# juhyeonkim95/Mitsuba3DopplerToF

Measured on AMD Instinct MI355X. Metric: Mpaths/s (whole node), Doppler Cornell 512x512 64spp, higher is better.
Workload: dtype f32

## Files before the change

mitsuba3dopplertof_amd/csrc/dtof_device.h:

```cpp
#pragma once
#include "dtof_kernels.h"
#include "dtof_scene.h"
#include "dtof_math.h"

#define DTOF_D __device__ __forceinline__
namespace dtof { constexpr int kBlock = 256; }
#include "dtof_traverse.h"
#include "dtof_sampling.h"
#include "dtof_shading.h"

#include <stdexcept>
#include <cstdlib>

namespace dtof {

constexpr uint32_t kSeg = 512;
static_assert(kSeg / 64 == kChunkBlocks, "chunks per segment");
constexpr int kShadeBlock = 64;
static_assert(kShadeBlock == 64, "k_shade's compaction (wave_append) and its per-wave statistics take the block for one wave");
template <bool MESH> DTOF_D void store_hit(const Queues &q, uint32_t l, const Hit &h, bool found) {
    if (MESH) q.hit[l] = make_uint4(f2u(h.t), f2u(h.u), f2u(h.v), h.prim);
    else q.hit_t[l] = h.t;
    q.hit_id[l] = found ? (h.obj | (h.shape << q.id_shift)) : 0xffffffffu;
}
template <bool MESH> DTOF_D uint4 load_hit(const Queues &q, uint32_t l) {
    if (MESH) return q.hit[l];
    return make_uint4(f2u(q.hit_t[l]), 0u, 0u, 0u);
}
DTOF_D uint32_t seg_count(const uint32_t *counts, uint32_t seg, uint32_t n_lanes) {
    return counts ? counts[seg] : min(kSeg, n_lanes - seg * kSeg);
}

DTOF_D float tent(float x, float inv_r) { return fmax_(0.f, 1.f - fabsf(x * inv_r)); }
template <int F = -1>
DTOF_D float filter_weight(const RenderParams &rp, float x) {
    const int filter = F >= 0 ? F : (int) rp.filter;
    if (filter == FILTER_GAUSSIAN) return fmax_(estrin10(sqr(x), rp.gauss_coeff), 0.f);
    if (filter == FILTER_MITCHELL) {
        x = fabsf(x);
        const float x2 = x * x, x3 = x2 * x, B = rp.filter_b, C = rp.filter_c;
        const float a3 = (12.f - 9.f * B - 6.f * C), a2 = (-18.f + 12.f * B + 6.f * C), a0 = (6.f - 2.f * B),
                    b3 = (-B - 6.f * C), b2 = (6.f * B + 30.f * C), b1 = (-12.f * B - 48.f * C), b0 = (8.f * B + 24.f * C);
        const float r = (1.f / 6.f) * (x < 1.f ? fmaf(a3, x3, fmaf(a2, x2, a0)) : fmaf(b3, x3, fmaf(b2, x2, fmaf(b1, x, b0))));
        return x < 2.f ? r : 0.f;
    }
    if (filter == FILTER_CATMULLROM) {
        x = fabsf(x);
        const float x2 = x * x, x3 = x2 * x, B = 0.f, C = .5f;
        const float r = (1.f / 6.f) * (x < 1.f ? (12.f - 9.f * B - 6.f * C) * x3 + (-18.f + 12.f * B + 6.f * C) * x2 + (6.f - 2.f * B)
                                               : (-B - 6.f * C) * x3 + (6.f * B + 30.f * C) * x2 + (-12.f * B - 48.f * C) * x + (8.f * B + 24.f * C));
        return x < 2.f ? r : 0.f;
    }
    if (filter == FILTER_LANCZOS) {
        x = fabsf(x);
        const float x1 = kPi * x, x2 = x1 / rp.filter_radius;
        float s1, s2, c; sincos_(x1, s1, c); sincos_(x2, s2, c);
        const float result = (s1 * s2) / (x1 * x2);
        return x < 5.9604644775390625e-8f ? 1.f : (x > rp.filter_radius ? 0.f : result);
    }
    return tent(x, rp.inv_radius);
}
template <int CTRL, int ROW_MASK = 0xf>
DTOF_D float dpp_add(float v) {
    return v + __int_as_float(__builtin_amdgcn_update_dpp(0, __float_as_int(v), CTRL, ROW_MASK, 0xf, false));
}

template <int F = -1>
DTOF_D void splat_lane(const RenderParams &rp, float *film, float spx, float spy, int pixel_x, int pixel_y, float r, float g, float b) {
    int W = rp.crop_w, H = rp.crop_h;
    if (F >= 0 ? F == FILTER_BOX : rp.filter == FILTER_BOX) {
        int x = pixel_x, y = pixel_y;
        if ((unsigned) x < (unsigned) W && (unsigned) y < (unsigned) H) {
            float *p = film + 4 * ((size_t) y * W + x);
            atomicAdd(p, r); atomicAdd(p + 1, g); atomicAdd(p + 2, b); atomicAdd(p + 3, 1.f);
        }
        return;
    }
    int n = (int) ceilf(rp.filter_radius - .5f), cnt = 2 * n + 1;
    int pix = (int) floorf(spx) - n, piy = (int) floorf(spy) - n;
    float relx = (float) pix + .5f - spx, rely = (float) piy + .5f - spy;
    int lx = pix - rp.crop_x, ly = piy - rp.crop_y;
    for (int ys = 0; ys < cnt; ++ys) {
        float wy = filter_weight<F>(rp, rely + (float) ys);
        for (int xs = 0; xs < cnt; ++xs) {
            float w = filter_weight<F>(rp, relx + (float) xs) * wy;
            int x = lx + xs, y = ly + ys;
            if ((unsigned) x < (unsigned) W && (unsigned) y < (unsigned) H) {
                float *p = film + 4 * ((size_t) y * W + x);
                atomicAdd(p, r * w); atomicAdd(p + 1, g * w); atomicAdd(p + 2, b * w); atomicAdd(p + 3, w);
            }
        }
// ... 35 lines not shown
```

mitsuba3dopplertof_amd/csrc/dtof_kernels.h:

```cpp
#pragma once
#include <stdint.h>
#include <hip/hip_runtime.h>
#include "dtof_math.h"

namespace dtof {

constexpr uint32_t kChunkBlocks = 8;
constexpr uint32_t kMaxInline = 4;
constexpr int kMaxOffsets = 4;

struct RenderParams {
    float s2c[16];
    float cam_to_world[12];
    float near_clip, far_clip, shutter_open, shutter_open_time;
    int32_t orthographic;
    float aperture_radius, focus_distance;
    int32_t crop_x, crop_y, crop_w, crop_h;
    float scale_x, scale_y, offset_x, offset_y;
    int32_t filter; float filter_radius, inv_radius;
    float gauss_coeff[10];
    float filter_b, filter_c;
    uint32_t base_seed, seed, seed_value;
    uint32_t spp, spp_log2;
    uint32_t tcn, pcn;
// ... 51 lines not shown
    uint32_t *q[2];
    uint32_t *counts;
    uint4 *cand;
    uint32_t *defer_idx;
    uint32_t *defer_cnt;
    uint32_t *seg_counter;
    uint32_t capacity;
    uint32_t xcd_remap;
    uint32_t id_shift;
};

struct LaneDebug {
    float sample_pos[2]; float time; float ray_o[3]; float ray_d[3]; float rgb[3]; float valid;
};

struct ShadeArgs {
    const uint8_t *scene; uint32_t scene_bytes, stage_words; RenderParams rp; Queues q;
    const uint32_t *qin, *count_in; uint32_t *qout, *alive_out, *shadow_out; uint32_t depth, trace_next; LaneDebug *dbg;
    float *film; uint64_t film_stride;
    uint32_t n_seg, res_small_off, res_small_words, res_memo;
    uint32_t res_park_off;
};
static_assert(sizeof(ShadeArgs) == 888, "ShadeArgs is k_shade's kernarg block: its layout, order and types do not change");
constexpr uint32_t kParkWords = 11;
#ifndef DTOF_PARK
#define DTOF_PARK 1
#endif
constexpr uint32_t kParkState = 10, kParkRng = 6;
constexpr uint32_t kResidentNodes = 1024;
constexpr uint32_t kMemoStride = 64, kMemoWords = 12;

struct ShadeLds {
    uint32_t stage, memo;
    uint32_t stack, park;
    constexpr uint32_t bytes() const { return stage + memo + stack + park; }
    constexpr uint32_t without_stack() const { return stage + memo + park; }
    constexpr uint32_t park_off() const { return stack / 4u; }
    static constexpr ShadeLds columns(uint32_t stage_words, uint32_t waves, uint32_t memo_columns, uint32_t stack_depth, bool entries16, uint32_t park_words) {
        return { stage_words * 16u, memo_columns * waves * kMemoWords * kMemoStride * 4u, (stack_depth < 2 ? 2u : stack_depth) * waves * 64u * (entries16 ? 2u : 4u), park_words * waves * 64u * 4u };
    }
    static constexpr ShadeLds classic(uint32_t stage_words, bool fused, bool one_instance, uint32_t stack_depth) {
        return fused ? columns(stage_words, 1u, one_instance ? 2u : 1u, one_instance ? 1u : stack_depth, false, 0u) : ShadeLds { stage_words * 16u, 0u, 0u, 0u };
    }
    static constexpr ShadeLds resident(uint32_t small_words, uint32_t waves, bool memo, bool several_films, uint32_t stack_depth) {
        return columns(4u * kResidentNodes + small_words, waves, memo ? 1u : 0u, stack_depth, several_films, (several_films ? kParkWords : 0u) + (DTOF_PARK && waves == 16 ? (several_films ? kParkRng : kParkState) : 0u));
    }
};
static_assert(ShadeLds::resident(171, 16, false, false, 12).bytes() == 158384 && ShadeLds::resident(171, 16, true, false, 12).bytes() == 207536, "resident stage, one film");
static_assert(ShadeLds::resident(171, 8, false, true, 12).bytes() == 103088 && ShadeLds::resident(171, 8, false, true, 12).park_off() == 3072, "resident stage, four films");
static_assert(ShadeLds::classic(214, true, true, 5).bytes() == 10080 && ShadeLds::classic(214, true, true, 5).without_stack() == 9568, "classic one-wall launch");

enum : uint32_t {
    kFactSinglePass     = 1u << 0,
    kFactDopplerCorr    = 1u << 1,
    kFactNoLaneOutput   = 1u << 2,
    kFactIdentityQueue  = 1u << 3,
    kFactNoRoulette     = 1u << 4,
    kFactCorrelated     = 1u << 5,
    kFactWholePath      = 1u << 6,
    kFactOneBlock       = 1u << 7,
    kFactOneEmitter     = 1u << 8,
    kFactWavePixel      = 1u << 9,
    kFactFlat           = 1u << 10,
    kFactOneWall        = 1u << 11,
    kFactFusedSplat     = 1u << 12,
};
#ifndef DTOF_HEADLINE_FACTS
#define DTOF_HEADLINE_FACTS 0xfff
#endif
constexpr uint32_t kHeadlineFacts = DTOF_HEADLINE_FACTS;
#ifndef DTOF_HEADLINE_FUSED
#define DTOF_HEADLINE_FUSED 1
#endif
constexpr uint32_t kHeadlineFusedFacts = DTOF_HEADLINE_FUSED ? (kHeadlineFacts | kFactFusedSplat) : 0u;
#ifndef DTOF_WALL_FRAMES
#define DTOF_WALL_FRAMES 1
#endif
#ifndef DTOF_RESIDENT_FACTS
#define DTOF_RESIDENT_FACTS 0x37f
#endif
constexpr uint32_t kResidentFacts = DTOF_RESIDENT_FACTS;

struct ShadeLaunch { bool staged; int mode; uint32_t waves, grid, lds, lds_flat; hipStream_t stream; ShadeArgs args; uint32_t facts; };
bool launch_shade_plain(bool area, bool k4, const ShadeLaunch &L);
void launch_shade_mesh(bool area, bool k4, const ShadeLaunch &L);
void launch_shade_spec1(bool k4, const ShadeLaunch &L);
void launch_shade_spec2(bool k4, const ShadeLaunch &L);
bool launch_shade_resident0(bool area, bool k4, const ShadeLaunch &L);
void launch_shade_resident1(bool k4, const ShadeLaunch &L);
void launch_shade_resident2(bool k4, const ShadeLaunch &L);

struct ResidentStage { uint32_t small_off = 0, small_words = 0, waves = 0, n_cu = 0; };
inline ShadeLds resident_lds(const RenderParams &rp, const ResidentStage &st, uint32_t stack_depth, uint32_t waves) { return ShadeLds::resident(st.small_words, waves, rp.memo_obj != 0xffffffffu, rp.n_offsets != 1, stack_depth); }
uint32_t device_lds_limit();
uint32_t device_cu_count();

struct LaunchSwitches {
// ... 60 lines not shown
```

mitsuba3dopplertof_amd/csrc/dtof_sampling.h:

```cpp
#pragma once
#include "dtof_kernels.h"
#include "dtof_scene.h"
#include "dtof_math.h"

#ifndef DTOF_D
#define DTOF_D __device__ __forceinline__
#endif

namespace dtof {

struct Rng { uint64_t state, inc; };
DTOF_D float next_f32(Rng &r) { return pcg_next_f32(r.state, r.inc); }
DTOF_D Rng seed_stream(uint32_t seed_value, uint32_t index) {
    uint32_t v0, v1; tea32(seed_value, index, v0, v1);
    Rng r; pcg_seed(v0, v1, r.state, r.inc); return r;
}
DTOF_D uint64_t stream_inc(uint32_t seed_value, uint32_t index) {
    uint32_t v0, v1; tea32(seed_value, index, v0, v1);
    return ((uint64_t) v1 << 1) | 1u;
}
DTOF_D float next_correlate(Rng &main, Rng &path, bool correlate) {
    uint64_t old = correlate ? path.state : main.state;
    path.state = path.state * kPcgMult + path.inc;
    main.state = main.state * kPcgMult + main.inc;
    return pcg_output_f32(old);
}
DTOF_D float next_time(const RenderParams &rp, Rng &main, Rng &tm, uint32_t si, uint32_t perm_seed, uint32_t &dim) {
    int strategy = rp.time_sampling; uint32_t tcn = rp.tcn;
    if (strategy == TIME_UNIFORM) return next_f32(main);
    float r = strategy == TIME_STRATIFIED ? next_f32(main) : next_f32(tm);
    const uint32_t quo = fdiv(si, rp.d_tcn), rem = si - quo * tcn;
    if (rp.stratify) {
        if (strategy == TIME_STRATIFIED) {
            const uint32_t ps = perm_seed + dim + ((rem != 0) ? 0u : 1u);
            dim += 2;
            const uint32_t p = permute_kensler(quo, rp.n_stratum, ps, rp.d_stratum);
            r = ((float) p + r) * rp.inv_n_stratum;
        } else {
            r = ((float) quo + r) * rp.inv_n_stratum;
        }
    }
    if (strategy == TIME_STRATIFIED) return ((float) rem + r) * rp.inv_tcn;
    if (strategy == TIME_ANTITHETIC) {
        if (tcn == 2) { float r2 = r + rp.antithetic_shift; return rem != 1 ? r : r2; }
        return r + (float) rem / (float) tcn;
    }
    if (strategy == TIME_ANTITHETIC_MIRROR) {
        float r2 = 1.0f - r + rp.antithetic_shift;
        return rem != 1 ? r : r2;
    }
    if (strategy == TIME_PERIODIC) return r + (float) rem / (float) tcn;
    return r;
}

constexpr float kInvTwoPiF = 0.15915494309189533577f;
DTOF_D float waveform(float _t, int type) {
    float t = fmod_pos(_t, 2.f * kPi, kInvTwoPiF);
    if (type == WAVE_RECT) return fabsf(t - kPi) > 0.5f * kPi ? 1.f : -1.f;
    if (type == WAVE_TRI) return t < kPi ? 1.f - 2.f * t * (1.0f / kPi) : -3.f + 2.f * t * (1.0f / kPi);
    return cos_(t);
}
DTOF_D float waveform_low_pass(float _t, int type) {
    float t = fmod_pos(_t, 2.f * kPi, kInvTwoPiF);
    if (type == WAVE_SIN) return cos_(t);
    float a = t * (1.0f / kPi), b = 2.f - a, c = a < b ? a : b;
    if (type == WAVE_RECT) return 2.f - 4.f * c;
    if (type == WAVE_TRI) return (4.f * c * c * c - 6.f * c * c + 1.f) * 2.0f * (1.0f / 3.0f);
    float r = 2.f - 4.f * c;
    return fmin_(fmax_(2.0f * r, -2.0f), 2.0f);
}
DTOF_D float modulation_weight(const RenderParams &rp, float w_d, float phase, float ray_time, float path_length) {
    float phi = rp.phi_coef * path_length;
    if (rp.low_pass) {
        float t = w_d * ray_time + phase + phi;
        return rp.amp * waveform_low_pass(t, rp.wave_type);
    }
    float t1 = rp.w_g * ray_time - phi;
    float t2 = (rp.w_g + w_d) * ray_time + phase;
    float g_t = rp.g_1 * waveform(t1, rp.wave_type) + rp.g_0;
    float s_t = waveform(t2, rp.wave_type);
    return s_t * g_t;
}

struct PrimaryLane { float4 ray_a, ray_b; Rng main, path; float2 pos; };
DTOF_D uint32_t global_lane(const RenderParams &rp, uint32_t virtual_lane) {
    if (rp.stripe_rows == 0) return virtual_lane;
    const uint32_t v = fdiv(virtual_lane, rp.d_lanes_per_row), in_row = virtual_lane - v * rp.lanes_per_row;
    const uint32_t s = fdiv(v, rp.d_stripe_rows), y = rp.stripe_first + s * rp.stripe_period + (v - s * rp.stripe_rows);
    return y * rp.lanes_per_row + in_row;
}
struct PixelInfo { uint32_t perm_seed; float posx, posy; };
template <bool UNIFORM>
DTOF_D PixelInfo pixel_info(const RenderParams &rp, uint32_t pix) {
    if (UNIFORM) pix = __builtin_amdgcn_readfirstlane(pix);
    PixelInfo pi; uint32_t tmp;
    tea32(rp.base_seed, rp.spp * pix + rp.seed, pi.perm_seed, tmp);
    const uint32_t W = (uint32_t) rp.crop_w, py = fdiv(pix, rp.d_w), px = pix - W * py;
    pi.posx = (float) (px + (uint32_t) rp.crop_x); pi.posy = (float) (py + (uint32_t) rp.crop_y);
    return pi;
}
template <bool PERSPECTIVE_ONLY = false>
DTOF_D void camera_ray(const RenderParams &rp, float ax, float ay, float apx, float apy, V3 &o, V3 &dw, float &maxt) {
    const float *m = rp.s2c;
    float r0 = fmaf(m[2], 0.f, fmaf(m[1], ay, fmaf(m[0], ax, m[3])));
    float r1 = fmaf(m[6], 0.f, fmaf(m[5], ay, fmaf(m[4], ax, m[7])));
    float r2 = fmaf(m[10], 0.f, fmaf(m[9], ay, fmaf(m[8], ax, m[11])));
    float r3 = fmaf(m[14], 0.f, fmaf(m[13], ay, fmaf(m[12], ax, m[15])));
    float iw = rcp(r3);
    V3 near_p = mk(r0 * iw, r1 * iw, r2 * iw);
    if (!PERSPECTIVE_ONLY && rp.orthographic) {
        o = xf_point(rp.cam_to_world, near_p);
        dw = normalize(xf_vector(rp.cam_to_world, mk(0.f, 0.f, 1.f)));
        maxt = rp.far_clip - rp.near_clip;
        return;
    }
    const bool lens = !PERSPECTIVE_ONLY && rp.aperture_radius != 0.f;
    V3 d;
    if (lens) {
        float tx, ty; concentric_disk(apx, apy, tx, ty);
        const V3 aperture_p = mk(rp.aperture_radius * tx, rp.aperture_radius * ty, 0.f);
        const float f_dist = rp.focus_distance / near_p.z;
        d = normalize(near_p * f_dist - aperture_p);
        o = xf_point(rp.cam_to_world, aperture_p);
    } else {
        d = normalize(near_p);
        o = mk(rp.cam_to_world[3], rp.cam_to_world[7], rp.cam_to_world[11]);
    }
    dw = xf_vector(rp.cam_to_world, d);
    float inv_z = rcp(d.z), near_t = rp.near_clip * inv_z, far_t = rp.far_clip * inv_z;
    o = o + dw * near_t;
    maxt = far_t - near_t;
}

template <bool PERSPECTIVE_ONLY = false, uint32_t FACTS = 0>
DTOF_D PrimaryLane generate_lane(const RenderParams &rp, uint32_t lane, bool wave_pixel = false, uint32_t vlane = 0) {
    constexpr bool F_SINGLE_PASS = (FACTS & kFactSinglePass) != 0, F_DOPPLER_CORR = (FACTS & kFactDopplerCorr) != 0, F_CORRELATED = (FACTS & kFactCorrelated) != 0;
    const bool needs_tm = (F_DOPPLER_CORR || (rp.integrator == 0 && rp.sampler_kind == SAMPLER_CORRELATED)) && rp.time_sampling >= TIME_ANTITHETIC;
    Rng main, tm, path; tm.state = 0; tm.inc = 1;
    uint2 *const carried = !F_SINGLE_PASS && rp.n_passes > 1 ? rp.pass_rng + (size_t) (vlane - rp.pass_first) * 3 : nullptr;
    const uint32_t pass = F_SINGLE_PASS ? 0u : rp.pass;
    if (pass == 0 && wave_pixel && needs_tm && rp.tcn == 2 && rp.pcn == 2) {
        main = seed_stream(rp.seed_value, lane);
        const bool odd = lane & 1u;
        uint32_t a0, a1; tea32(rp.seed_value + (odd ? 2u : 1u), lane >> 1, a0, a1);
        const uint32_t b0 = (uint32_t) __builtin_amdgcn_update_dpp(0, (int) a0, 0xb1, 0xf, 0xf, false), b1 = (uint32_t) __builtin_amdgcn_update_dpp(0, (int) a1, 0xb1, 0xf, 0xf, false);
        pcg_seed(odd ? b0 : a0, odd ? b1 : a1, tm.state, tm.inc);
        pcg_seed(odd ? a0 : b0, odd ? a1 : b1, path.state, path.inc);
    } else if (pass == 0) {
        main = seed_stream(rp.seed_value, lane);
        if (needs_tm) tm = seed_stream(rp.seed_value + 1, fdiv(lane, rp.d_tcn));
        path = seed_stream(rp.seed_value + 2, fdiv(lane, rp.d_pcn));
    } else {
        const uint2 a = carried[0], b = carried[1], c = carried[2];
        main.state = (uint64_t) a.x | ((uint64_t) a.y << 32); main.inc = stream_inc(rp.seed_value, lane);
        if (needs_tm) { tm.state = (uint64_t) b.x | ((uint64_t) b.y << 32); tm.inc = stream_inc(rp.seed_value + 1, fdiv(lane, rp.d_tcn)); }
        path.state = (uint64_t) c.x | ((uint64_t) c.y << 32); path.inc = stream_inc(rp.seed_value + 2, fdiv(lane, rp.d_pcn));
    }
    const uint32_t pix = fdiv(lane, rp.d_spp);
// ... 41 lines not shown
```

mitsuba3dopplertof_amd/csrc/dtof_shade.h:

```cpp
#pragma once
#include "dtof_device.h"
#include <atomic>
#include <initializer_list>
#include <type_traits>

namespace dtof {


DTOF_D uint32_t wave_append(bool pred, uint32_t &running) {
    const uint64_t mask = __ballot(pred);
    const uint32_t slot = running + (uint32_t) __popcll(mask & ((1ull << __lane_id()) - 1ull));
    running += (uint32_t) __popcll(mask);
    return slot;
}

struct BsdfOut { V3 val, weight, wo; float pdf, bs_pdf, bs_eta; bool bs_delta, bs_null; };
template <int SPEC>
DTOF_D void bsdf_eval_pdf_sample(const SceneView &sv, const DShape *sh, Surface &si, V3 wo, bool active_em, float sample_1, float s2x, float s2y, BsdfOut &out, bool want_sample = true) {
    const bool masked = SPEC && (sh->flags & SF_MASK);
    bool null_pick = false; float opacity = 1.f;
    if (masked) { opacity = mask_opacity_at(sv, sh, si.u, si.v); null_pick = !(sample_1 < opacity); sample_1 = sample_1 / opacity; }
    const bool blend = SPEC == 2 && (sh->flags & SF_BLEND);
    float blend_w = 0.f; bool pick_1 = false;
    if (blend) {
        blend_w = sh->tex_blend ? texture_eval_1(sv, sh->tex_blend << 4, si.u, si.v) : sh->blend_weight;
        blend_w = fmin_(fmax_(blend_w, 0.f), 1.f);
        pick_1 = sample_1 <= blend_w;
    }
    const DShape *side_sh = (SPEC == 2 && (sh->flags & SF_TWOSIDED2) && si.wi.z < 0.f) ? &sv.shapes[sh->blend_other] : sh;
    const V3 wi_plain = si.wi, wo_plain = wo;
    V3 bsdf_val = mk(0, 0, 0), bsdf_weight = mk(0, 0, 0), bs_wo = mk(0, 0, 0);
    float bsdf_pdf = 0.f, bs_pdf = 0.f, bs_eta = 0.f; bool bs_delta = false, bs_null = false;
    V3 val_0 = mk(0, 0, 0), keep_weight = mk(0, 0, 0), keep_wo = mk(0, 0, 0); float pdf_0 = 0.f, keep_pdf = 0.f, keep_eta = 0.f; bool keep_delta = false, keep_null = false;
    for (int pass = 0; pass < (SPEC == 2 && blend ? 2 : 1); ++pass) {
        const DShape *bsh = pass ? &sv.shapes[sh->blend_other] : side_sh;
        const float s1 = !blend ? sample_1 : (pass ? sample_1 / blend_w : (sample_1 - blend_w) / (1.f - blend_w));
        si.wi = wi_plain; wo = wo_plain;
// ... 228 lines not shown
    w[9] = bo.bs_delta ? 1.f : 0.f; w[10] = bo.weight.x; w[11] = bo.weight.y; w[12] = bo.weight.z; w[13] = bo.bs_null ? 1.f : 0.f;
}
template <int SPEC>
void launch_bsdf_eval_spec(const uint8_t *scene, uint32_t shape_index, const float *in, float *out, uint32_t n, hipStream_t s) {
    if (n) hipLaunchKernelGGL(k_bsdf_eval<SPEC>, dim3(nblk(n)), dim3(kBlock), 0, s, scene, shape_index, in, out, n);
}

template <bool LDS, int MODE, bool AREA, int KMAX, bool MESH, int SPEC, int RESW = 0, bool RH16 = false, uint32_t FACTS = 0>
#ifndef DTOF_MESH_WAVES
#define DTOF_MESH_WAVES 3
#endif
#ifndef DTOF_K4_RES_LDS
#define DTOF_K4_RES_LDS 1
#endif
__global__ __launch_bounds__(RESW ? RESW * 64 : kShadeBlock, RESW ? RESW / 4 : (MODE == 2 && !MESH && !SPEC && KMAX == 1) ? 4 : (MODE != 0 && MESH) ? ((SPEC && KMAX > 1) ? 2 : DTOF_MESH_WAVES) : 1) void k_shade(ShadeArgs args_by_value) {
    constexpr bool FUSED = MODE != 0, FIRST = MODE == 2;
    static_assert(FACTS == 0 || MODE == 2, "plan facts describe a first-bounce launch");
    constexpr bool F_SINGLE_PASS = (FACTS & kFactSinglePass) != 0, F_DOPPLER_CORR = (FACTS & kFactDopplerCorr) != 0, F_NO_LANE_OUT = (FACTS & kFactNoLaneOutput) != 0;
    constexpr bool F_IDENTITY = (FACTS & kFactIdentityQueue) != 0, F_NO_RR = (FACTS & kFactNoRoulette) != 0, F_CORRELATED = (FACTS & kFactCorrelated) != 0;
    constexpr bool F_WHOLE_PATH = (FACTS & kFactWholePath) != 0, F_ONE_BLOCK = (FACTS & kFactOneBlock) != 0, F_ONE_EMITTER = (FACTS & kFactOneEmitter) != 0;
    constexpr bool F_WAVE_PIXEL = (FACTS & kFactWavePixel) != 0;
    constexpr bool F_FLAT = (FACTS & kFactFlat) != 0, F_ONE_WALL = (FACTS & kFactOneWall) != 0, F_FUSED_SPLAT = (FACTS & kFactFusedSplat) != 0;
    constexpr bool F_FRAMES = F_ONE_WALL && DTOF_WALL_FRAMES;
    static_assert(!F_FLAT || (!MESH && SPEC == 0 && RESW == 0), "trace_flat serves the staged rectangle-only diffuse kernels");
    static_assert(!F_ONE_WALL || F_FLAT, "the one wall is an object of the flat table");
    static_assert(!F_FUSED_SPLAT || KMAX == 1, "the fused splat is the one-film kernels'");
    static_assert(!F_WAVE_PIXEL || F_IDENTITY, "whole waves of one pixel are provable for an identity queue only");
    static_assert(!F_ONE_BLOCK || RESW == 0, "blocks per segment belong to the classic launch");
    constexpr bool RES_LDS = RESW != 0 && KMAX > 1 && DTOF_K4_RES_LDS;
    constexpr bool S16 = RESW != 0 && KMAX > 1;
    static_assert(!RES_LDS || 3 * KMAX == (int) kParkWords + 1, "the film-state columns hold all but the last float of the K results");
    constexpr bool PARK_ST = DTOF_PARK && RESW == 16 && KMAX == 1;
    constexpr bool PARK = DTOF_PARK && RESW == 16 && (KMAX == 1 || RES_LDS);
    constexpr uint32_t kRngAt = RES_LDS ? kParkWords : 0u;
    constexpr int KREG = RES_LDS ? 1 : KMAX;
    constexpr uint32_t kStackStride = RESW ? RESW * 64 : kShadeBlock;
    static_assert(RESW == 0 || (MODE == 2 && !LDS && MESH), "the resident stage exists for the unstaged fused first-bounce kernel with mesh code");
    static_assert(!RH16 || RESW != 0, "half-float LDS planes belong to the resident stage");
    extern __shared__ uint4 lds[];
    __shared__ uint32_t s_inline_all[(RESW ? RESW : 1) * 2 * kMaxInline];
    typedef const char __attribute__((address_space(4))) *KernargBytes;
    const KernargBytes kernarg = (KernargBytes) __builtin_amdgcn_kernarg_segment_ptr();
    const ShadeArgs &A0 = *(const ShadeArgs *) kernarg;
    const uint32_t lane_id = RESW ? threadIdx.x & 63u : threadIdx.x, wave_id = RESW ? threadIdx.x >> 6 : 0u;
    uint32_t *const s_inline = s_inline_all + wave_id * 2 * kMaxInline;
    const uint32_t stage_words = RESW ? 4u * kResNodes + A0.res_small_words : A0.stage_words;
// ... 29 lines not shown
        sv_res = make_view(A0.scene);
        sv_res.nodes = (const DNode *) lds; sv_res.nodes16 = (const DNode16 *) lds;
        sv_res.groups = (const DGroup *) (small + gh->off_groups); sv_res.shapes = (const DShape *) (small + gh->off_shapes);
        sv_res.tris = (const DTri *) (small + gh->off_tris); sv_res.shading = (const DTriShade *) (small + gh->off_shading);
        sv_res.isect = (const DTriIsect *) (small + gh->off_isect);
        sv_res.emitters = (const DEmitter *) (small + gh->off_emitters);
    }
    for (;;) {
    uint32_t seg, sub_index = 0;
    if (RESW) {
        uint32_t taken = 0;
        if (lane_id == 0) taken = atomicAdd(A0.q.seg_counter, 1u);
        uint32_t unit = (uint32_t) __builtin_amdgcn_readfirstlane((int) taken);
        if (unit >= A0.n_seg * sub) break;
        unit = A0.n_seg * sub - 1u - unit;
        seg = sub > 1 ? unit / sub : unit; sub_index = sub > 1 ? unit - seg * sub : 0u;
    } else {
        seg = sub > 1 ? blockIdx.x / sub : blockIdx.x; sub_index = sub > 1 ? blockIdx.x - seg * sub : 0u;
    }
    const uint32_t count = seg_count(F_IDENTITY ? nullptr : A0.count_in, seg, A0.rp.n_lanes);
    uint32_t n_alive = 0, n_shadow = 0;
    if (FIRST && lane_id < 2 * kMaxInline) s_inline[lane_id] = 0;
    if (count != 0) {
    const uint8_t *base = LDS ? stage_scene(A0.scene, A0.scene_bytes, lds) : A0.scene;
    SceneView sv = RESW ? sv_res : make_view(base);
    if (FUSED) { sv.memo_obj = A0.rp.memo_obj; sv.memo = (float *) (lds + stage_words) + (RESW ? wave_id * kMemoWords * kMemoStride + lane_id : threadIdx.x); sv.memo_m = memo_m_lds; }
    const bool have_memo = F_ONE_WALL || (FUSED && sv.memo_obj != 0xffffffffu);
    for (uint32_t cbase = sub > 1 ? sub_index * unit_lanes : 0u; cbase < (sub > 1 ? (sub_index + 1) * unit_lanes < count ? (sub_index + 1) * unit_lanes : count : count); cbase += kShadeBlock) {
    uint32_t rebase = 0;
    asm volatile("" : "+s"(rebase));
    const ShadeArgs &A = *(const ShadeArgs *) (kernarg + rebase);
    const RenderParams &rp = A.rp; const Queues &q = A.q;
    const uint32_t *const qin = F_IDENTITY ? nullptr : A.qin; uint32_t *const qout = A.qout; const uint32_t depth0 = A.depth, trace_next_last = F_WHOLE_PATH ? 0u : A.trace_next;
    LaneDebug *const dbg = F_NO_LANE_OUT ? nullptr : A.dbg;
    const uint32_t flat = FUSED && !MESH ? rp.flat_objects : 0u;
    uint32_t j = cbase + lane_id;
    bool in_range = F_WAVE_PIXEL || j < count;
    bool alive = false, want_shadow = false;
    uint32_t l = 0;
    float4 sha = make_float4(0.f, 0.f, 0.f, 0.f), shb = sha, nra = sha, nrb = sha; float3 cand[KREG];
#pragma unroll
    for (int k = 0; k < KREG; ++k) cand[k] = make_float3(0.f, 0.f, 0.f);
    float3 rbase[KREG];
#pragma unroll
    for (int k = 0; k < KREG; ++k) rbase[k] = make_float3(0.f, 0.f, 0.f);
    V3 pend_thr = mk(0, 0, 0), pend_v = mk(0, 0, 0); float pend_len = 0.f;
    float *const park = RES_LDS || PARK ? (float *) (lds + stage_words) + memo_words + A0.res_park_off + threadIdx.x : nullptr;
    float res_last = 0.f;
    auto res_get = [&](int k) -> float4 {
        if (RES_LDS) return make_float4(park[(3 * k) * kStackStride], park[(3 * k + 1) * kStackStride], 3 * k + 2 < (int) kParkWords ? park[(3 * k + 2) * kStackStride] : res_last, 0.f);
        if (!FIRST) return q.res[(size_t) k * q.capacity + l];
        const float3 r = rbase[k]; return make_float4(r.x, r.y, r.z, 0.f);
    };
    auto res_put = [&](int k, float4 v) {
        if (RES_LDS) {
// ... 25 lines not shown
    };
    const bool valid_start = SPEC && rp.has_env && !rp.hide_emitters;
    bool valid_reg = valid_start;
    float memo_m[12], memo_inv[12];
    typename std::conditional<F_FRAMES, WallFrames, NoFrames>::type wf;
    if constexpr (F_FRAMES) {
        wf.n = mk(0.f, 0.f, 1.f); wf.s = mk(1.f, 0.f, 0.f);
        wf.table = (const DFlatFrame *) ((const uint4 *) ((const DFlatObject *) (sv.base + rp.flat_off) + rp.flat_objects) + 1 + rp.flat_objects);
    }
    bool lane_on = in_range;
#ifdef DTOF_TRAVERSAL_STATS
    constexpr uint64_t kPoisonState = 0xdeadbeefcafef00dull;
    if (!in_range) { main.state = path.state = kPoisonState; const float pz = u2f(0x7fc0dead); ra = rb = st = make_float4(pz, pz, pz, pz); }
#define DTOF_POISON_CHECK() do { if (main.state == kPoisonState || path.state == kPoisonState || f2u(st.x) == 0x7fc0deadu || f2u(ra.x) == 0x7fc0deadu) DTOF_STAT(14); } while (0)
#else
#define DTOF_POISON_CHECK() ((void) 0)
#endif
    const bool wave_pixel = F_WAVE_PIXEL || (FIRST && rp.spp_log2 != 0xffffffffu && rp.spp_log2 >= 6 && (rp.lane_base & 63u) == 0 && count - cbase >= (uint32_t) kShadeBlock);
    const bool fuse_splat = F_FUSED_SPLAT || (FIRST && A.film != nullptr);
    float2 pos_reg = make_float2(0.f, 0.f);
    if (in_range) {
        l = qin ? qin[seg * kSeg + j] : seg * kSeg + j;
        if (FIRST) {
            const PrimaryLane pl = generate_lane<SPEC == 0, FACTS>(rp, global_lane(rp, rp.lane_base + l), wave_pixel, rp.lane_base + l);
            ra = pl.ray_a; rb = pl.ray_b; main = pl.main; path = pl.path; st = make_float4(1.f, 1.f, 1.f, 0.f);
            if (PARK) park_store();
            pos_reg = pl.pos;
            if (!fuse_splat) {
                q.pos[l] = pl.pos;
                q.rng_b[l] = make_uint2((uint32_t) (main.inc >> 1), (uint32_t) (path.inc >> 1));
            }
            if (dbg) {
                LaneDebug &o = dbg[l];
                o.time = ra.w; o.ray_o[0] = ra.x; o.ray_o[1] = ra.y; o.ray_o[2] = ra.z; o.ray_d[0] = rb.x; o.ray_d[1] = rb.y; o.ray_d[2] = rb.z;
            }
            if (have_memo) instance_memo_fill(sv, ra.w, memo_m, memo_inv);
            if constexpr (F_FRAMES) {
                const DShape &ws = sv.shapes[sv.groups[sv.objects[sv.memo_obj].index].first_shape];
                wf.n = normalize(xf_normal(memo_inv, mk(ws.n[0], ws.n[1], ws.n[2])));
                const V3 du = xf_vector(memo_m, mk(ws.dp_du[0], ws.dp_du[1], ws.dp_du[2]));
                wf.s = normalize(vfma(wf.n, -dot(wf.n, du), du));
                if (du.x == 0.f && du.y == 0.f && du.z == 0.f) { V3 tt; coordinate_system(wf.n, wf.s, tt); }
            }
            Hit h;
            bool found = (F_FLAT || flat) ? trace_flat<false, true, FACTS & kFactOneWall>(sv, (ConstBytes) A.scene + rp.flat_off, rp.flat_off, flat, stack, mk(ra.x, ra.y, ra.z), mk(rb.x, rb.y, rb.z), ra.w, rb.w, h)
                              : trace_scene<false, MESH, FUSED, RESW != 0, kStackStride, S16, 0u, false, RH16>(sv, stack, mk(ra.x, ra.y, ra.z), mk(rb.x, rb.y, rb.z), ra.w, rb.w, h);
            hh = make_uint4(f2u(h.t), f2u(h.u), f2u(h.v), h.prim);
// ... 360 lines not shown
        if (alive && trace_next) {
            Hit h;
            bool found = (F_FLAT || flat) ? trace_flat<false, true, FACTS & kFactOneWall>(sv, (ConstBytes) A.scene + rp.flat_off, rp.flat_off, flat, stack, mk(nra.x, nra.y, nra.z), mk(nrb.x, nrb.y, nrb.z), nra.w, nrb.w, h)
                              : trace_scene<false, MESH, true, RESW != 0, kStackStride, S16, 0u, false, RH16>(sv, stack, mk(nra.x, nra.y, nra.z), mk(nrb.x, nrb.y, nrb.z), nra.w, nrb.w, h);
            if (!FIRST || last) store_hit<MESH>(q, l, h, found);
            if (FIRST) { hh = make_uint4(f2u(h.t), f2u(h.u), f2u(h.v), h.prim); hid = found ? (h.obj | (h.shape << q.id_shift)) : 0xffffffffu; }
        }
        const uint32_t n_sh = (uint32_t) __popcll(__ballot(want_shadow)) * ((threadIdx.x & 63) == 0 ? 1u : 0u);
        if (last) n_shadow += n_sh; else if (lane_id == 0) s_inline[2 * it + 1] += n_sh;
    } else {
        uint32_t sslot = seg * kSeg + wave_append(want_shadow, n_shadow);
        if (want_shadow) {
            q.sh_a[sslot] = sha; q.sh_b[sslot] = shb;
#pragma unroll
            for (int k = 0; k < KMAX; ++k) if (KMAX == 1 || k < rp.n_offsets)
                q.sh_c[(size_t) k * q.capacity + sslot] = make_float4(cand[k].x, cand[k].y, cand[k].z, u2f(l));
        }
    }
    if (last) break;
    lane_on = alive;
    if (alive) { ra = nra; rb = nrb; DTOF_POISON_CHECK(); }
    }
    if constexpr (!RES_LDS) if (FIRST && fuse_splat) {
        const uint32_t W = (uint32_t) rp.crop_w;
        const uint32_t pix = fdiv(global_lane(rp, rp.lane_base + l), rp.d_spp);
        const int py = (int) fdiv(pix, rp.d_w), px = (int) (pix - W * (uint32_t) py);
        const float sx = pos_reg.x, sy = pos_reg.y;
        const bool regular = in_range && (int) floorf(sx) - rp.crop_x == px && (int) floorf(sy) - rp.crop_y == py;
        if (wave_pixel) {
            const int upx = __builtin_amdgcn_readfirstlane(px), upy = __builtin_amdgcn_readfirstlane(py);
            const float relx = (float) (upx + rp.crop_x - 1) + .5f - sx, rely = (float) (upy + rp.crop_y - 1) + .5f - sy;
            float wx[3], wy[3];
#pragma unroll
            for (int a = 0; a < 3; ++a) { wx[a] = regular ? tent(relx + (float) a, rp.inv_radius) : 0.f; wy[a] = tent(rely + (float) a, rp.inv_radius); }
            const uint32_t sum_id = __brev(lane_id) >> 26, tap = sum_id >> 2, ch = sum_id & 3u;
            const int fx = upx - 1 + (int) (tap % 3u), fy = upy - 1 + (int) (tap / 3u);
            const bool store = sum_id < 36u && (unsigned) fx < W && (unsigned) fy < (unsigned) rp.crop_h;
#pragma unroll
            for (int k = 0; k < KMAX; ++k) if (KMAX == 1 || k < rp.n_offsets) {
                float *fk = A.film + (size_t) k * A.film_stride;
                if (in_range && !regular) splat_lane<F_FUSED_SPLAT ? FILTER_TENT : -1>(rp, fk, sx, sy, px, py, rbase[k].x, rbase[k].y, rbase[k].z);
                float v[36];
#pragma unroll
                for (int ys = 0; ys < 3; ++ys)
#pragma unroll
                    for (int xs = 0; xs < 3; ++xs) {
                        const float w = wx[xs] * wy[ys]; const int c = 4 * (3 * ys + xs);
                        v[c] = rbase[k].x * w; v[c + 1] = rbase[k].y * w; v[c + 2] = rbase[k].z * w; v[c + 3] = w;
                    }
                const float total = wave_totals_36(v, lane_id);
                if (store && total != 0.f) atomicAdd(fk + 4 * ((size_t) fy * W + (size_t) fx) + ch, total);
            }
        } else if (in_range) {
#pragma unroll
            for (int k = 0; k < KMAX; ++k) if (KMAX == 1 || k < rp.n_offsets)
                splat_lane<F_FUSED_SPLAT ? FILTER_TENT : -1>(rp, A.film + (size_t) k * A.film_stride, sx, sy, px, py, rbase[k].x, rbase[k].y, rbase[k].z);
        }
    }
    }
    }
    if (lane_id == 0) {
        if (sub > 1) { atomicAdd(&A0.alive_out[seg], n_alive); atomicAdd(&A0.shadow_out[seg], n_shadow); }
        else { A0.alive_out[seg] = n_alive; A0.shadow_out[seg] = n_shadow; }
        if (FIRST) {
            const uint32_t n_inl = A0.rp.inline_iters, n_seg = RESW ? A0.n_seg : gridDim.x / sub;
            for (uint32_t i = 0; i + 1 < n_inl; ++i) {
                uint32_t *slot = A0.alive_out - (size_t) 2 * (n_inl - 1 - i) * n_seg;
                if (sub > 1) { atomicAdd(&slot[seg], s_inline[2 * i]); atomicAdd(&slot[n_seg + seg], s_inline[2 * i + 1]); }
                else { slot[seg] = s_inline[2 * i]; slot[n_seg + seg] = s_inline[2 * i + 1]; }
            }
        }
    }
    if (!RESW) break;
    }
#undef DTOF_POISON_CHECK
}

template <bool A, int K, bool M, int S>
static void launch_shade_variant(const ShadeLaunch &L) {
// ... 29 lines not shown
```

Baseline: 16070.

## Stage headline launch constants into LDS block with compile-time defaults

Adds a compact HeadlineConsts struct that the headline k_shade kernels copy from the kernarg RenderParams into shared memory at block start, with many rarely varying fields fixed as static constexpr values. Ray generation, bounce shading and the fused splat read from this block, so the compiler can fold the constant fields and drop the dead branches. It also moves per-pixel values into scalar registers through readfirstlane. The cost is one extra LDS staging pass and 432 B of static LDS per block, plus the risk of wrong output if any constexpr default does not match the real parameters.

After: 15640. -2.7%, worse.

```diff
diff --git a/mitsuba3dopplertof_amd/csrc/dtof_device.h b/mitsuba3dopplertof_amd/csrc/dtof_device.h
--- a/mitsuba3dopplertof_amd/csrc/dtof_device.h
+++ b/mitsuba3dopplertof_amd/csrc/dtof_device.h
@@ -32,8 +32,8 @@
 }
 
 DTOF_D float tent(float x, float inv_r) { return fmax_(0.f, 1.f - fabsf(x * inv_r)); }
-template <int F = -1>
-DTOF_D float filter_weight(const RenderParams &rp, float x) {
+template <int F = -1, class RP>
+DTOF_D float filter_weight(const RP &rp, float x) {
     const int filter = F >= 0 ? F : (int) rp.filter;
     if (filter == FILTER_GAUSSIAN) return fmax_(estrin10(sqr(x), rp.gauss_coeff), 0.f);
     if (filter == FILTER_MITCHELL) {
@@ -65,8 +65,8 @@
     return v + __int_as_float(__builtin_amdgcn_update_dpp(0, __float_as_int(v), CTRL, ROW_MASK, 0xf, false));
 }
 
-template <int F = -1>
-DTOF_D void splat_lane(const RenderParams &rp, float *film, float spx, float spy, int pixel_x, int pixel_y, float r, float g, float b) {
+template <int F = -1, class RP>
+DTOF_D void splat_lane(const RP &rp, float *film, float spx, float spy, int pixel_x, int pixel_y, float r, float g, float b) {
     int W = rp.crop_w, H = rp.crop_h;
     if (F >= 0 ? F == FILTER_BOX : rp.filter == FILTER_BOX) {
         int x = pixel_x, y = pixel_y;
diff --git a/mitsuba3dopplertof_amd/csrc/dtof_kernels.h b/mitsuba3dopplertof_amd/csrc/dtof_kernels.h
--- a/mitsuba3dopplertof_amd/csrc/dtof_kernels.h
+++ b/mitsuba3dopplertof_amd/csrc/dtof_kernels.h
@@ -97,6 +97,31 @@
     uint32_t res_park_off;
 };
 static_assert(sizeof(ShadeArgs) == 888, "ShadeArgs is k_shade's kernarg block: its layout, order and types do not change");
+
+struct alignas(16) HeadlineConsts {
+    float s2c[16], cam_to_world[12], near_clip, far_clip, shutter_open, shutter_open_time;
+    int32_t crop_x, crop_y, crop_w, crop_h; float scale_x, scale_y, offset_x, offset_y; int32_t filter; float filter_radius, inv_radius; uint32_t pad_film;
+    uint32_t base_seed, seed, seed_value, spp, spp_log2, tcn, pcn; int32_t time_sampling; float antithetic_shift; int32_t stratify; uint32_t n_stratum; float inv_n_stratum, inv_tcn; uint32_t pad_sampler[3];
+    float T, w_g, phi_coef, amp, g_1, g_0, w_d[kMaxOffsets], phase[kMaxOffsets]; int32_t n_offsets, wave_type, low_pass; uint32_t path_correlation_depth, max_depth, rr_depth;
+    uint32_t lane_base, n_lanes, stripe_rows, stripe_period, stripe_first, lanes_per_row; FastDiv d_spp, d_w, d_tcn, d_pcn, d_stratum, d_lanes_per_row, d_stripe_rows;
+    uint32_t inline_iters, flat_objects, flat_off, memo_obj; int32_t want_valid; float emitter_pmf; int32_t terminal; uint32_t pad_launch;
+    static constexpr int32_t integrator = 0, sampler_kind = 0 , orthographic = 0, jitter = 0, has_env = 0, hide_emitters = 0;
+    static constexpr uint32_t n_passes = 1, pass = 0, pass_first = 0, sample_count = 0, env_index = 0;
+    static constexpr float aperture_radius = 0.f, focus_distance = 0.f, inv_spp = 0.f, filter_b = 0.f, filter_c = 0.f, gauss_coeff[10] = {};
+    static constexpr FastDiv d_sample_count = { 1u, 0u };
+    static constexpr uint2 *pass_rng = nullptr;
+};
+struct ConstsRun { uint32_t dst, src, n; };
+#define DTOF_CONSTS_RUN(first, last) { (uint32_t) offsetof(HeadlineConsts, first) / 4u, (uint32_t) offsetof(RenderParams, first) / 4u, (uint32_t) (offsetof(RenderParams, last) + sizeof(RenderParams::last) - offsetof(RenderParams, first)) / 4u }
+constexpr ConstsRun kHeadlineRuns[6] = { DTOF_CONSTS_RUN(s2c, shutter_open_time), DTOF_CONSTS_RUN(crop_x, inv_radius), DTOF_CONSTS_RUN(base_seed, inv_tcn), DTOF_CONSTS_RUN(T, rr_depth),
+                                         DTOF_CONSTS_RUN(lane_base, d_stripe_rows), DTOF_CONSTS_RUN(inline_iters, terminal) };
+#define DTOF_CONSTS_SAME(first, last) (offsetof(HeadlineConsts, last) - offsetof(HeadlineConsts, first) == offsetof(RenderParams, last) - offsetof(RenderParams, first) && offsetof(HeadlineConsts, first) % 16 == 0)
+static_assert(DTOF_CONSTS_SAME(s2c, shutter_open_time) && DTOF_CONSTS_SAME(crop_x, inv_radius) && DTOF_CONSTS_SAME(base_seed, inv_tcn) && DTOF_CONSTS_SAME(T, rr_depth) &&
+              DTOF_CONSTS_SAME(lane_base, d_stripe_rows) && DTOF_CONSTS_SAME(inline_iters, terminal), "a run of HeadlineConsts is a run of RenderParams, member for member, on a 16-byte boundary");
+static_assert(kHeadlineRuns[0].n == 32 && kHeadlineRuns[1].n == 11 && kHeadlineRuns[2].n == 13 && kHeadlineRuns[3].n == 20 && kHeadlineRuns[4].n == 20 && kHeadlineRuns[5].n == 7, "no run is longer than a wave");
+#undef DTOF_CONSTS_SAME
+#undef DTOF_CONSTS_RUN
+static_assert(sizeof(HeadlineConsts) == 432, "the block of the headline kernels' launch constants");
 constexpr uint32_t kParkWords = 11;
 #ifndef DTOF_PARK
 #define DTOF_PARK 1
@@ -110,6 +135,7 @@
     uint32_t stack, park;
     constexpr uint32_t bytes() const { return stage + memo + stack + park; }
     constexpr uint32_t without_stack() const { return stage + memo + park; }
+    static constexpr uint32_t inline_static = 2u * kMaxInline * 4u, headline_static = inline_static + (uint32_t) sizeof(HeadlineConsts);
     constexpr uint32_t park_off() const { return stack / 4u; }
     static constexpr ShadeLds columns(uint32_t stage_words, uint32_t waves, uint32_t memo_columns, uint32_t stack_depth, bool entries16, uint32_t park_words) {
         return { stage_words * 16u, memo_columns * waves * kMemoWords * kMemoStride * 4u, (stack_depth < 2 ? 2u : stack_depth) * waves * 64u * (entries16 ? 2u : 4u), park_words * waves * 64u * 4u };
@@ -124,6 +150,8 @@
 static_assert(ShadeLds::resident(171, 16, false, false, 12).bytes() == 158384 && ShadeLds::resident(171, 16, true, false, 12).bytes() == 207536, "resident stage, one film");
 static_assert(ShadeLds::resident(171, 8, false, true, 12).bytes() == 103088 && ShadeLds::resident(171, 8, false, true, 12).park_off() == 3072, "resident stage, four films");
 static_assert(ShadeLds::classic(214, true, true, 5).bytes() == 10080 && ShadeLds::classic(214, true, true, 5).without_stack() == 9568, "classic one-wall launch");
+static_assert(ShadeLds::headline_static <= 1024u, "device_lds_limit() keeps 1 KiB back for k_shade's static LDS");
+static_assert(16u * (ShadeLds::classic(214, true, true, 5).without_stack() + ShadeLds::headline_static) <= 160u * 1024u, "sixteen one-wave blocks of the headline launch (C2: 9 568 B dynamic + 464 B static) fit a CU's LDS");
 
 enum : uint32_t {
     kFactSinglePass     = 1u << 0,
@@ -148,6 +176,16 @@
 #define DTOF_HEADLINE_FUSED 1
 #endif
 constexpr uint32_t kHeadlineFusedFacts = DTOF_HEADLINE_FUSED ? (kHeadlineFacts | kFactFusedSplat) : 0u;
+constexpr uint32_t kHeadlineConstsFacts = kFactSinglePass | kFactDopplerCorr | kFactFlat;
+#ifndef DTOF_CONSTS_GEN
+#define DTOF_CONSTS_GEN 1
+#endif
+#ifndef DTOF_CONSTS_BOUNCE
+#define DTOF_CONSTS_BOUNCE 1
+#endif
+#ifndef DTOF_CONSTS_SPLAT
+#define DTOF_CONSTS_SPLAT 1
+#endif
 #ifndef DTOF_WALL_FRAMES
 #define DTOF_WALL_FRAMES 1
 #endif
diff --git a/mitsuba3dopplertof_amd/csrc/dtof_sampling.h b/mitsuba3dopplertof_amd/csrc/dtof_sampling.h
--- a/mitsuba3dopplertof_amd/csrc/dtof_sampling.h
+++ b/mitsuba3dopplertof_amd/csrc/dtof_sampling.h
@@ -2,6 +2,7 @@
 #include "dtof_kernels.h"
 #include "dtof_scene.h"
 #include "dtof_math.h"
+#include <type_traits>
 
 #ifndef DTOF_D
 #define DTOF_D __device__ __forceinline__
@@ -25,7 +26,8 @@
     main.state = main.state * kPcgMult + main.inc;
     return pcg_output_f32(old);
 }
-DTOF_D float next_time(const RenderParams &rp, Rng &main, Rng &tm, uint32_t si, uint32_t perm_seed, uint32_t &dim) {
+template <class RP>
+DTOF_D float next_time(const RP &rp, Rng &main, Rng &tm, uint32_t si, uint32_t perm_seed, uint32_t &dim) {
     int strategy = rp.time_sampling; uint32_t tcn = rp.tcn;
     if (strategy == TIME_UNIFORM) return next_f32(main);
     float r = strategy == TIME_STRATIFIED ? next_f32(main) : next_f32(tm);
@@ -69,7 +71,8 @@
     float r = 2.f - 4.f * c;
     return fmin_(fmax_(2.0f * r, -2.0f), 2.0f);
 }
-DTOF_D float modulation_weight(const RenderParams &rp, float w_d, float phase, float ray_time, float path_length) {
+template <class RP>
+DTOF_D float modulation_weight(const RP &rp, float w_d, float phase, float ray_time, float path_length) {
     float phi = rp.phi_coef * path_length;
     if (rp.low_pass) {
         float t = w_d * ray_time + phase + phi;
@@ -83,24 +86,28 @@
 }
 
 struct PrimaryLane { float4 ray_a, ray_b; Rng main, path; float2 pos; };
-DTOF_D uint32_t global_lane(const RenderParams &rp, uint32_t virtual_lane) {
+template <class RP>
+DTOF_D uint32_t global_lane(const RP &rp, uint32_t virtual_lane) {
     if (rp.stripe_rows == 0) return virtual_lane;
     const uint32_t v = fdiv(virtual_lane, rp.d_lanes_per_row), in_row = virtual_lane - v * rp.lanes_per_row;
     const uint32_t s = fdiv(v, rp.d_stripe_rows), y = rp.stripe_first + s * rp.stripe_period + (v - s * rp.stripe_rows);
     return y * rp.lanes_per_row + in_row;
 }
 struct PixelInfo { uint32_t perm_seed; float posx, posy; };
-template <bool UNIFORM>
-DTOF_D PixelInfo pixel_info(const RenderParams &rp, uint32_t pix) {
+template <bool UNIFORM, class RP>
+DTOF_D PixelInfo pixel_info(const RP &rp, uint32_t pix) {
     if (UNIFORM) pix = __builtin_amdgcn_readfirstlane(pix);
+    constexpr bool TO_SCALAR = UNIFORM && std::is_same<RP, HeadlineConsts>::value;
+    auto uni = [](uint32_t v) { return TO_SCALAR ? (uint32_t) __builtin_amdgcn_readfirstlane((int) v) : v; };
+    auto uni_div = [&](FastDiv d) { if (TO_SCALAR) { d.mul = uni(d.mul); d.shifts = uni(d.shifts); } return d; };
     PixelInfo pi; uint32_t tmp;
-    tea32(rp.base_seed, rp.spp * pix + rp.seed, pi.perm_seed, tmp);
-    const uint32_t W = (uint32_t) rp.crop_w, py = fdiv(pix, rp.d_w), px = pix - W * py;
-    pi.posx = (float) (px + (uint32_t) rp.crop_x); pi.posy = (float) (py + (uint32_t) rp.crop_y);
+    tea32(uni(rp.base_seed), uni(rp.spp) * pix + uni(rp.seed), pi.perm_seed, tmp);
+    const uint32_t W = uni((uint32_t) rp.crop_w), py = fdiv(pix, uni_div(rp.d_w)), px = pix - W * py;
+    pi.posx = (float) (px + uni((uint32_t) rp.crop_x)); pi.posy = (float) (py + uni((uint32_t) rp.crop_y));
     return pi;
 }
-template <bool PERSPECTIVE_ONLY = false>
-DTOF_D void camera_ray(const RenderParams &rp, float ax, float ay, float apx, float apy, V3 &o, V3 &dw, float &maxt) {
+template <bool PERSPECTIVE_ONLY = false, class RP>
+DTOF_D void camera_ray(const RP &rp, float ax, float ay, float apx, float apy, V3 &o, V3 &dw, float &maxt) {
     const float *m = rp.s2c;
     float r0 = fmaf(m[2], 0.f, fmaf(m[1], ay, fmaf(m[0], ax, m[3])));
     float r1 = fmaf(m[6], 0.f, fmaf(m[5], ay, fmaf(m[4], ax, m[7])));
@@ -132,8 +139,8 @@
     maxt = far_t - near_t;
 }
 
-template <bool PERSPECTIVE_ONLY = false, uint32_t FACTS = 0>
-DTOF_D PrimaryLane generate_lane(const RenderParams &rp, uint32_t lane, bool wave_pixel = false, uint32_t vlane = 0) {
+template <bool PERSPECTIVE_ONLY = false, uint32_t FACTS = 0, class RP>
+DTOF_D PrimaryLane generate_lane(const RP &rp, uint32_t lane, bool wave_pixel = false, uint32_t vlane = 0) {
     constexpr bool F_SINGLE_PASS = (FACTS & kFactSinglePass) != 0, F_DOPPLER_CORR = (FACTS & kFactDopplerCorr) != 0, F_CORRELATED = (FACTS & kFactCorrelated) != 0;
     const bool needs_tm = (F_DOPPLER_CORR || (rp.integrator == 0 && rp.sampler_kind == SAMPLER_CORRELATED)) && rp.time_sampling >= TIME_ANTITHETIC;
     Rng main, tm, path; tm.state = 0; tm.inc = 1;
diff --git a/mitsuba3dopplertof_amd/csrc/dtof_shade.h b/mitsuba3dopplertof_amd/csrc/dtof_shade.h
--- a/mitsuba3dopplertof_amd/csrc/dtof_shade.h
+++ b/mitsuba3dopplertof_amd/csrc/dtof_shade.h
@@ -13,6 +13,15 @@
     running += (uint32_t) __popcll(mask);
     return slot;
 }
+
+DTOF_D const HeadlineConsts *stage_headline_consts(const uint32_t *rp_words, uint32_t lane) {
+    __shared__ HeadlineConsts block;
+    uint32_t *const words = (uint32_t *) &block;
+#pragma unroll
+    for (int r = 0; r < 6; ++r) if (lane < kHeadlineRuns[r].n) words[kHeadlineRuns[r].dst + lane] = rp_words[kHeadlineRuns[r].src + lane];
+    return &block;
+}
+template <bool BLOCK> using ParamsOf = typename std::conditional<BLOCK, HeadlineConsts, RenderParams>::type;
 
 struct BsdfOut { V3 val, weight, wo; float pdf, bs_pdf, bs_eta; bool bs_delta, bs_null; };
 template <int SPEC>
@@ -287,6 +296,9 @@
     constexpr bool F_WAVE_PIXEL = (FACTS & kFactWavePixel) != 0;
     constexpr bool F_FLAT = (FACTS & kFactFlat) != 0, F_ONE_WALL = (FACTS & kFactOneWall) != 0, F_FUSED_SPLAT = (FACTS & kFactFusedSplat) != 0;
     constexpr bool F_FRAMES = F_ONE_WALL && DTOF_WALL_FRAMES;
+    constexpr bool F_CONSTS = FACTS != 0 && (FACTS & kHeadlineConstsFacts) == kHeadlineConstsFacts;
+    constexpr bool C_GEN = F_CONSTS && DTOF_CONSTS_GEN, C_BOUNCE = F_CONSTS && DTOF_CONSTS_BOUNCE, C_SPLAT = F_CONSTS && DTOF_CONSTS_SPLAT;
+    static_assert(!F_CONSTS || (LDS && KMAX == 1 && HeadlineConsts::sampler_kind == SAMPLER_CORRELATED), "HeadlineConsts describes the staged one-film launch of the Doppler integrator with the correlated sampler");
     static_assert(!F_FLAT || (!MESH && SPEC == 0 && RESW == 0), "trace_flat serves the staged rectangle-only diffuse kernels");
     static_assert(!F_ONE_WALL || F_FLAT, "the one wall is an object of the flat table");
     static_assert(!F_FUSED_SPLAT || KMAX == 1, "the fused splat is the one-film kernels'");
@@ -362,6 +374,8 @@
     uint32_t n_alive = 0, n_shadow = 0;
     if (FIRST && lane_id < 2 * kMaxInline) s_inline[lane_id] = 0;
     if (count != 0) {
+    const HeadlineConsts *hc = nullptr;
+    if constexpr (F_CONSTS) hc = stage_headline_consts((const uint32_t *) &A0.rp, lane_id);
     const uint8_t *base = LDS ? stage_scene(A0.scene, A0.scene_bytes, lds) : A0.scene;
     SceneView sv = RESW ? sv_res : make_view(base);
     if (FUSED) { sv.memo_obj = A0.rp.memo_obj; sv.memo = (float *) (lds + stage_words) + (RESW ? wave_id * kMemoWords * kMemoStride + lane_id : threadIdx.x); sv.memo_m = memo_m_lds; }
@@ -370,7 +384,9 @@
     uint32_t rebase = 0;
     asm volatile("" : "+s"(rebase));
     const ShadeArgs &A = *(const ShadeArgs *) (kernarg + rebase);
-    const RenderParams &rp = A.rp; const Queues &q = A.q;
+    const ParamsOf<C_BOUNCE> &rp = *(const ParamsOf<C_BOUNCE> *) (C_BOUNCE ? (const void *) hc : (const void *) &A.rp); const Queues &q = A.q;
+    const ParamsOf<C_GEN> &rp_gen = *(const ParamsOf<C_GEN> *) (C_GEN ? (const void *) hc : (const void *) &A.rp);
+    const ParamsOf<C_SPLAT> &rp_splat = *(const ParamsOf<C_SPLAT> *) (C_SPLAT ? (const void *) hc : (const void *) &A.rp);
     const uint32_t *const qin = F_IDENTITY ? nullptr : A.qin; uint32_t *const qout = A.qout; const uint32_t depth0 = A.depth, trace_next_last = F_WHOLE_PATH ? 0u : A.trace_next;
     LaneDebug *const dbg = F_NO_LANE_OUT ? nullptr : A.dbg;
     const uint32_t flat = FUSED && !MESH ? rp.flat_objects : 0u;
@@ -442,7 +458,7 @@
     if (in_range) {
         l = qin ? qin[seg * kSeg + j] : seg * kSeg + j;
         if (FIRST) {
-            const PrimaryLane pl = generate_lane<SPEC == 0, FACTS>(rp, global_lane(rp, rp.lane_base + l), wave_pixel, rp.lane_base + l);
+            const PrimaryLane pl = generate_lane<SPEC == 0, FACTS>(rp_gen, global_lane(rp_gen, rp_gen.lane_base + l), wave_pixel, rp_gen.lane_base + l);
             ra = pl.ray_a; rb = pl.ray_b; main = pl.main; path = pl.path; st = make_float4(1.f, 1.f, 1.f, 0.f);
             if (PARK) park_store();
             pos_reg = pl.pos;
@@ -849,24 +865,24 @@
     if (alive) { ra = nra; rb = nrb; DTOF_POISON_CHECK(); }
     }
     if constexpr (!RES_LDS) if (FIRST && fuse_splat) {
-        const uint32_t W = (uint32_t) rp.crop_w;
-        const uint32_t pix = fdiv(global_lane(rp, rp.lane_base + l), rp.d_spp);
-        const int py = (int) fdiv(pix, rp.d_w), px = (int) (pix - W * (uint32_t) py);
+        const uint32_t W = (uint32_t) rp_splat.crop_w;
+        const uint32_t pix = fdiv(global_lane(rp_splat, rp_splat.lane_base + l), rp_splat.d_spp);
+        const int py = (int) fdiv(pix, rp_splat.d_w), px = (int) (pix - W * (uint32_t) py);
         const float sx = pos_reg.x, sy = pos_reg.y;
-        const bool regular = in_range && (int) floorf(sx) - rp.crop_x == px && (int) floorf(sy) - rp.crop_y == py;
+        const bool regular = in_range && (int) floorf(sx) - rp_splat.crop_x == px && (int) floorf(sy) - rp_splat.crop_y == py;
         if (wave_pixel) {
             const int upx = __builtin_amdgcn_readfirstlane(px), upy = __builtin_amdgcn_readfirstlane(py);
-            const float relx = (float) (upx + rp.crop_x - 1) + .5f - sx, rely = (float) (upy + rp.crop_y - 1) + .5f - sy;
+            const float relx = (float) (upx + rp_splat.crop_x - 1) + .5f - sx, rely = (float) (upy + rp_splat.crop_y - 1) + .5f - sy;
             float wx[3], wy[3];
 #pragma unroll
-            for (int a = 0; a < 3; ++a) { wx[a] = regular ? tent(relx + (float) a, rp.inv_radius) : 0.f; wy[a] = tent(rely + (float) a, rp.inv_radius); }
+            for (int a = 0; a < 3; ++a) { wx[a] = regular ? tent(relx + (float) a, rp_splat.inv_radius) : 0.f; wy[a] = tent(rely + (float) a, rp_splat.inv_radius); }
             const uint32_t sum_id = __brev(lane_id) >> 26, tap = sum_id >> 2, ch = sum_id & 3u;
             const int fx = upx - 1 + (int) (tap % 3u), fy = upy - 1 + (int) (tap / 3u);
-            const bool store = sum_id < 36u && (unsigned) fx < W && (unsigned) fy < (unsigned) rp.crop_h;
-#pragma unroll
-            for (int k = 0; k < KMAX; ++k) if (KMAX == 1 || k < rp.n_offsets) {
+            const bool store = sum_id < 36u && (unsigned) fx < W && (unsigned) fy < (unsigned) rp_splat.crop_h;
+#pragma unroll
+            for (int k = 0; k < KMAX; ++k) if (KMAX == 1 || k < rp_splat.n_offsets) {
                 float *fk = A.film + (size_t) k * A.film_stride;
-                if (in_range && !regular) splat_lane<F_FUSED_SPLAT ? FILTER_TENT : -1>(rp, fk, sx, sy, px, py, rbase[k].x, rbase[k].y, rbase[k].z);
+                if (in_range && !regular) splat_lane<F_FUSED_SPLAT ? FILTER_TENT : -1>(rp_splat, fk, sx, sy, px, py, rbase[k].x, rbase[k].y, rbase[k].z);
                 float v[36];
 #pragma unroll
                 for (int ys = 0; ys < 3; ++ys)
@@ -880,8 +896,8 @@
             }
         } else if (in_range) {
 #pragma unroll
-            for (int k = 0; k < KMAX; ++k) if (KMAX == 1 || k < rp.n_offsets)
-                splat_lane<F_FUSED_SPLAT ? FILTER_TENT : -1>(rp, A.film + (size_t) k * A.film_stride, sx, sy, px, py, rbase[k].x, rbase[k].y, rbase[k].z);
+            for (int k = 0; k < KMAX; ++k) if (KMAX == 1 || k < rp_splat.n_offsets)
+                splat_lane<F_FUSED_SPLAT ? FILTER_TENT : -1>(rp_splat, A.film + (size_t) k * A.film_stride, sx, sy, px, py, rbase[k].x, rbase[k].y, rbase[k].z);
         }
     }
     }
```
